# blachlylab/fade

Hardware: AMD Instinct MI355X
Metric: annotate reads/sec at 1/2/4/8 MI355X; rs/am tag bit-exact vs ref (higher is better)
Workload: dtype int16; 1 GPU; C2: 10000000 x 150 bp PE reads per GPU per step in 10 distinct batches, -w 100, --min-length 5, p_softclip 0.10; slots_in_flight=2, records_left_out=none

## Files before the change

### fade_amd/csrc/fadehip.hip

```cpp
#include "fadehip_host.hpp"
#include "fadehip_kernels.hpp"
#include "sw_stats.hpp"
#include <fcntl.h>
#include <sys/stat.h>
#include <unistd.h>
#include <algorithm>
#include <cerrno>
#include <climits>
#include <cstdio>
#include <cstdlib>
#include <cstring>
#include <string>
#include <thread>
#include <vector>

using namespace fadehip;
using namespace fadehip::host;

namespace {

int reserve_run(fadehip_ctx *ctx, std::vector<void *> &trash, DevBuf &b, size_t bytes) {
    if (bytes <= b.cap && b.p) return 0;
    if (b.p) trash.push_back(b.p);
    b.p = nullptr;
// ... 83 lines not shown
    return 0;
}

constexpr int SW_INT32 = -1;
template <int C = 0>
const void *sw_kernel(int cls, int mode, bool longw) {
    if constexpr (C >= NUM_CLASSES) {
        return nullptr;
    } else {
        if (cls != C) return sw_kernel<C + 1>(cls, mode, longw);
        constexpr int R = class_rows(C);
        switch (mode) {
        case SW_INT32: return (const void *)sw_forward_kernel<R>;
        case 0: return longw ? (const void *)sw_pk_kernel<R, 0, true> : (const void *)sw_pk_kernel<R, 0>;
        case 1: return longw ? (const void *)sw_pk_kernel<R, 1, true> : (const void *)sw_pk_kernel<R, 1>;
        case 2: return longw ? (const void *)sw_pk_kernel<R, 2, true> : (const void *)sw_pk_kernel<R, 2>;
        default: return longw ? (const void *)sw_pk_kernel<R, 3, true> : (const void *)sw_pk_kernel<R, 3>;
        }
    }
}

const void *sw64_kernel(int R) {
    switch (R) {
    case 12: return (const void *)sw_forward64_kernel<12>;
    case 16: return (const void *)sw_forward64_kernel<16>;
    case 24: return (const void *)sw_forward64_kernel<24>;
    case 32: return (const void *)sw_forward64_kernel<32>;
    case 48: return (const void *)sw_forward64_kernel<48>;
    default: return (const void *)sw_forward64_kernel<64>;
    }
}

template <int R8>
const void *g8_pick(const fadehip_ctx *ctx, int steps, bool *framed) {
    const ScoreTab &sc = ctx->sc;
    *framed = ctx->score_frame && frame_fits(std::max(std::max(sc.match, sc.mismatch), 0), sc.open, sc.ext, 8 * R8, steps);
    return *framed ? (const void *)sw_pk_kernel<R8, 1, false, 8, false, 0, true> : (const void *)sw_pk_kernel<R8, 1, false, 8>;
}
const void *g8_kernel(const fadehip_ctx *ctx, int cls, int max_lq, int steps, bool *framed) {
    const int score_g8 = ctx->score_g8, rows16 = 16 * class_rows(cls);
    *framed = false;
    if (!score_g8 || max_lq > rows16) return nullptr;
    if (max_lq <= 40 && rows16 > 40) return g8_pick<5>(ctx, steps, framed);
    if (max_lq <= 56 && rows16 > 56) return g8_pick<7>(ctx, steps, framed);
    if (max_lq <= 80 && rows16 > 80) return g8_pick<10>(ctx, steps, framed);
    if (max_lq <= 104 && rows16 > 104) return g8_pick<13>(ctx, steps, framed);
    if (max_lq <= 152 && rows16 > 152 && rows16 <= 160)
        return score_g8 == 2 ? (const void *)sw_pk_kernel<19, 1, false, 8, false, 2> : g8_pick<19>(ctx, steps, framed);
    return nullptr;
}

int launch_sw(fadehip_ctx *ctx, const void *fn, int grid, size_t lds, hipStream_t st, SwArgs a) {
    void *args[] = {&a};
    HIPCHK(ctx, hipLaunchKernel(fn, dim3((unsigned)grid), dim3(64), args, lds, st));
    return 0;
}

int resident_waves(fadehip_ctx *ctx, int cls, int mode, size_t lds, bool longw) {
    const uint64_t key = ((uint64_t)cls << 40) | ((uint64_t)mode << 32) | ((uint64_t)longw << 36) | (uint64_t)lds;
    std::lock_guard<std::mutex> l(ctx->resident_mu);
    auto it = ctx->resident.find(key);
    if (it != ctx->resident.end()) return it->second;
    int per_cu = 0;
    const void *fn = sw_kernel(cls, mode, longw);
    if (!fn || hipOccupancyMaxActiveBlocksPerMultiprocessor(&per_cu, fn, 64, lds) != hipSuccess || per_cu <= 0) per_cu = 4;
    const int w = per_cu * std::max(ctx->cu_count, 1);
    ctx->resident[key] = w;
    return w;
}

struct ClassRun {
    int cls = 0;
    const Work *work = nullptr;
    const Meta *meta = nullptr;
// ... 78 lines not shown
    p.mode2 = alt_rules ? 3 : 2;
    const int64_t ck_bytes = (int64_t)p.ck_stride * 4;
    p.total_oct = (n_items + 7) / 8;
    p.chunk_oct = std::max<int64_t>(1, std::min<int64_t>(p.total_oct, (c.budget / 2) / std::max<int64_t>(ck_bytes, 1)));
    p.wave_stride = (uint64_t)p.n_blocks1 * R * 64;
    p.longw = p.n_blocks1 > CH_BLOCKS;
    const int resident = resident_waves(ctx, cls, p.mode2, p.lds1, p.longw);
    const int bound_waves = (int)std::min<int64_t>(p.chunk_oct + NUM_BUCKETS, resident);
    int p2_waves = s.p2_last_octs[cls] >= 0 ? std::min(2 * s.p2_last_octs[cls] + 64, bound_waves) : std::min(1024, bound_waves);
    if (ctx->p2_waves_fixed > 0) p2_waves = std::min(ctx->p2_waves_fixed, bound_waves);
    p.p2_waves = (int)std::max<int64_t>(1, std::min<int64_t>(p2_waves, (c.budget / 2) / std::max<int64_t>((int64_t)p.wave_stride * 4, 1)));
    p.ckpt_bytes = (size_t)(p.chunk_oct * ck_bytes);
    p.fwd_bytes = (size_t)n_items * sizeof(Fwd);
    p.trace_bytes = (size_t)p.p2_waves * (size_t)p.wave_stride * 4;
    p.cand_bytes = sizeof(Cand) * (size_t)NUM_BUCKETS * (size_t)std::min<int64_t>(n_items, p.chunk_oct * 8);
    return 0;
}

constexpr size_t PATCH_ZB_OFF = sizeof(PatchHead), PATCH_LIST_OFF = PATCH_ZB_OFF + Slot::ZB_STRIDE;
static_assert(PATCH_LIST_OFF % 16 == 0 && Slot::ZB_BYTES % 4 == 0, "the gather copies dwords; entries stay 16-byte aligned");

int run_class_two_pass(fadehip_ctx *ctx, Slot &s, hipStream_t st, const ClassRun &c) {
    const int cls = c.cls, n_items = c.n_bound;
    TwoPassPlan p;
    int rc;
    if ((rc = plan_two_pass(ctx, s, c, p))) return rc;
    if ((rc = reserve_run(ctx, s.trash, s.ckpt, p.ckpt_bytes)) || (rc = reserve_run(ctx, s.trash, s.fwd, p.fwd_bytes)) ||
        (rc = reserve_run(ctx, s.trash, s.trace, p.trace_bytes)) || (rc = reserve_run(ctx, s.trash, s.cand, p.cand_bytes)))
        return rc;
    s.prof_counts[2] = std::max<int64_t>(s.prof_counts[2], (int64_t)p.trace_bytes);
    uint32_t *const sel_counters = s.d_sel(cls);
    const void *const score_fn = sw_kernel(cls, 1, p.longw), *const trace_fn = sw_kernel(cls, p.mode2, p.longw);
    if (!score_fn || !trace_fn) return set_err(ctx, FADEHIP_E_INVALID, "bad class %d", cls);
    bool framed = false;
    const void *const g8_fn = !p.longw && p.n_ck == 0 ? g8_kernel(ctx, cls, s.max_lq, 4 * p.n_blocks1, &framed) : nullptr;
    if (p.total_oct > p.chunk_oct) s.early = false;
    const bool early = s.early;
    for (int64_t o0 = 0; o0 < p.total_oct; o0 += p.chunk_oct) {
        const int octs = (int)std::min<int64_t>(p.chunk_oct, p.total_oct - o0);
        const int i0 = (int)(o0 * 8);
        const int n = std::min(n_items - i0, octs * 8);
        if (!s.sel_fresh[cls]) HIPCHK(ctx, hipMemsetAsync(sel_counters, 0, sizeof(uint32_t) * NUM_BUCKETS, st));
        s.sel_fresh[cls] = false;
        SwArgs a = sw_args(ctx, s, c, i0, n);
        a.ref_stride = p.ref_stride1;
        a.ckpt = (uint32_t *)s.ckpt.p;
        a.ck_stride = p.ck_stride;
        a.n_ck = p.n_ck;
        a.count_dev = c.count_dev;
        a.item_base = (uint32_t)i0;
        a.sel.enabled = 1;
        a.sel.no_ckpt = p.n_ck == 0 ? 1 : 0;
        a.sel.meta = c.meta ? c.meta + i0 : nullptr;
        a.sel.floor_len = c.floor_len;
        a.sel.trace_all = ctx->prm.trace_all;
        a.sel.span_slack = ctx->span_slack;
        a.sel.cand = (Cand *)s.cand.p;
        a.sel.cap = (uint32_t)n;
        a.sel.bucket_n = sel_counters;
        a.sel.out = c.out;
        a.sel.rs = c.rs;
        a.sel.stats = (c.rs && c.gate) ? s.d_stats() : nullptr;
        a.sel.gate = c.gate;
        a.sel.match = getenv("FADEHIP_NO_SHORTCUT") ? 0 : ctx->sc.match;
        a.sel.mismatch = ctx->sc.mismatch;
        hipStream_t sst = s.score_stream ? s.score_stream : st;
        if (sst != st) {
            int ef = -1;
            if ((rc = record(ctx, s, &ef, st))) return rc;
            HIPCHK(ctx, hipStreamWaitEvent(sst, s.ev[ef], 0));
        }
        ChunkSpans sp{c.timed};
        if ((rc = sp.mark(ctx, s, 0, sst))) return rc;
        const void *fn1 = score_fn;
        int waves1 = octs;
        size_t lds = p.lds1;
        if (ctx->score_persist && class_rows(cls) == 10 && !p.longw && s.tickets_used < (int)Slot::N_TICKETS) {
            const int res = resident_waves(ctx, cls, 1, p.lds1, p.longw);
            const int cus = std::max(ctx->cu_count, 1), mine = s.score_stream ? std::max(cus - 8 * ctx->tail_cus_per_xcd, 1) : cus;
            fn1 = (const void *)sw_pk_kernel<10, 1, false, 16, true>;
            waves1 = std::max(1, std::min(octs, (int)((int64_t)res * mine / cus)));
            a.ticket = s.d_ticket(s.tickets_used++);
        } else if (g8_fn) {
            if (ctx->debug && o0 == 0) fprintf(stderr, "[fadehip] class of %d rows: score pass on eight-lane groups (longest read of the batch: %d), column-drift frame %s\n", 16 * class_rows(cls), s.max_lq, framed ? "on" : "off");
            fn1 = g8_fn;
            waves1 = (n + 15) / 16;
            lds = 2 * p.lds1;
        }
        if ((rc = launch_sw(ctx, fn1, waves1, lds, sst, a))) return rc;
        if ((rc = sp.mark(ctx, s, 1, sst))) return rc;
        hipStream_t p2st = st;
        if (sst != st || early) {
            int ej = sp.e[1];
            if (ej < 0 && (rc = record(ctx, s, &ej, sst))) return rc;
            if (sst != st) HIPCHK(ctx, hipStreamWaitEvent(st, s.ev[ej], 0));
            if (early) {
                if (s.tail_stream) {
                    p2st = s.tail_stream;
                    HIPCHK(ctx, hipStreamWaitEvent(p2st, s.ev[ej], 0));
                }
                HIPCHK(ctx, hipMemcpyAsync(s.res.p + s.res_aln_off, s.aln.p, sizeof(fadehip_aln) * (size_t)s.out_cap, hipMemcpyDeviceToHost,
                                           s.tail_stream ? st : sst));
                HIPCHK(ctx, hipMemcpyAsync(s.res.p, c.rs, (size_t)s.n_reads, hipMemcpyDeviceToHost, s.tail_stream ? st : sst));
            }
        }
        if (s.tickets_used >= (int)Slot::N_TICKETS)
            return set_err(ctx, FADEHIP_E_UNSUPPORTED, "more than %d pass-2 launches in one run (raise trace_bytes)", (int)Slot::N_TICKETS);
        SwArgs b2 = a;
        b2.sel.enabled = 0;
        b2.n_items = 0;
        b2.cand = (const Cand *)s.cand.p;
        b2.cand_cap = (uint32_t)n;
        b2.bucket_n = sel_counters;
        b2.cand_total = &s.d_plan()->cand_total;
        b2.trace = (uint32_t *)s.trace.p;
        b2.quad_stride = p.wave_stride;
        b2.count_dev = nullptr;
// ... 1406 lines not shown
```

### fade_amd/csrc/fadehip_ctx.hip

```cpp
#include "fadehip_host.hpp"
#include <rccl/rccl.h>
#include <algorithm>
#include <cstdarg>
#include <cstdio>
#include <cstdlib>
#include <cstring>
#include <ctime>
#include <new>
#include <unordered_map>

using namespace fadehip;
using namespace fadehip::host;

namespace {

thread_local std::string g_err = "";
thread_local const fadehip_ctx *g_err_ctx = nullptr;

constexpr size_t PIN_REGISTER_MIN = (size_t)1 << 20;
std::mutex g_pin_mu;
std::unordered_map<void *, bool> g_pin_registered;

int pin_alloc(fadehip_ctx *ctx, size_t bytes, void **out) {
    *out = nullptr;
// ... 189 lines not shown
        if (atoi(kv)) {
            ctx->blocking_sync = true;
            (void)hipSetDevice(device);
            if (hipSetDeviceFlags(hipDeviceScheduleBlockingSync) != hipSuccess) (void)hipGetLastError();
        }
    }
    hipDeviceProp_t prop;
    if (hipSetDevice(device) != hipSuccess || hipGetDeviceProperties(&prop, device) != hipSuccess) {
        set_err(ctx, FADEHIP_E_NODEVICE, "cannot open HIP device %d", device);
        return fail(FADEHIP_E_NODEVICE);
    }
    if (strncmp(prop.gcnArchName, "gfx950", 6) != 0) {
        set_err(ctx, FADEHIP_E_NODEVICE, "device %d is %s; this library carries gfx950 code only", device, prop.gcnArchName);
        return fail(FADEHIP_E_NODEVICE);
    }
    ctx->cu_count = prop.multiProcessorCount;
    if (const char *kv = getenv("FADEHIP_KERNEL")) {
        ctx->use_packed = strcmp(kv, "int32") != 0;
        ctx->two_pass = strcmp(kv, "twopass") == 0;
    }
    if (ctx->prm.match > 2) ctx->two_pass = false;
    if (8 * (ctx->prm.match * FADEHIP_MAX_QUERY + ctx->prm.open + std::max(ctx->prm.match, 0)) >= 0x7c00) ctx->use_packed = false;
    if (!ctx->two_pass && ctx->prm.rules != FADEHIP_RULES_DEFAULT) {
        set_err(ctx, FADEHIP_E_UNSUPPORTED, "the rule switches exist on the two-pass path only (match <= 2, FADEHIP_KERNEL unset)");
        return fail(FADEHIP_E_UNSUPPORTED);
    }
    if (const char *kv = getenv("FADEHIP_SPAN_SLACK")) ctx->span_slack = atoi(kv);
    if (const char *kv = getenv("FADEHIP_TAIL_CUS")) ctx->tail_cus_per_xcd = std::max(0, std::min(atoi(kv), 8));
    if (const char *kv = getenv("FADEHIP_BAM_SPLIT")) ctx->split_cus = std::max(0, std::min(atoi(kv), 31));
    if (const char *kv = getenv("FADEHIP_P2_WAVES")) ctx->p2_waves_fixed = std::max(0, atoi(kv));
    if (const char *kv = getenv("FADEHIP_SCORE_PERSIST")) ctx->score_persist = atoi(kv) != 0;
    if (const char *kv = getenv("FADEHIP_SCORE_G8")) ctx->score_g8 = atoi(kv);
    if (const char *kv = getenv("FADEHIP_SCORE_FRAME")) ctx->score_frame = atoi(kv) != 0;
    if (const char *kv = getenv("FADEHIP_EARLY_COPY")) ctx->early_copy = atoi(kv) != 0;
    if (const char *kv = getenv("FADEHIP_EARLY_TAIL")) ctx->early_tail = strcmp(kv, "masked") == 0 ? 1 : strcmp(kv, "plain") == 0 ? 2 : 0;
    if (const char *kv = getenv("FADEHIP_PATCH_CAP")) ctx->patch_cap = std::max(0, std::min(atoi(kv), 1 << 20));
    ctx->debug = getenv("FADEHIP_DEBUG") != nullptr;
    if (hipStreamCreateWithFlags(&ctx->copy_stream, hipStreamNonBlocking) != hipSuccess ||
        upload_ascii_code(ctx->copy_stream) != hipSuccess) {
        set_err(ctx, FADEHIP_E_HIP, "hipMemcpyToSymbol failed: %s", hipGetErrorString(hipGetLastError()));
        return fail(FADEHIP_E_HIP);
    }
    for (int k = 0; k < FADEHIP_NUM_SLOTS; k++)
        for (int c = 0; c < NUM_CLASSES; c++) ctx->slots[k].p2_last_octs[c] = -1;
    *out = ctx;
    return 0;
}

void fadehip_destroy(fadehip_ctx *ctx) {
    if (!ctx) return;
    (void)hipSetDevice(ctx->device);
    (void)hipDeviceSynchronize();
    for (int k = 0; k < FADEHIP_NUM_SLOTS; k++) {
        Slot &s = ctx->slots[k];
        for (DevBuf *b : {&s.in[0], &s.in[1], &s.rs, &s.fwd, &s.aln, &s.zblock, &s.trace, &s.ckpt, &s.cand, &s.lrows}) release(*b);
        for (void *q : s.trash) (void)hipFree(q);
        s.trash.clear();
        for (int c = 0; c < NUM_LISTS; c++) {
            release(s.work[c]);
            release(s.meta[c]);
        }
        release(s.stage[0]);
        release(s.stage[1]);
        release(s.res);
        release(s.patch);
        release(s.h_patch);
// ... 179 lines not shown
```

### fade_amd/csrc/fadehip_host.hpp

```cpp
#pragma once
#include <hip/hip_runtime.h>
#include <climits>
#include <cstdint>
#include <map>
#include <mutex>
#include <string>
#include <vector>
#include "../../include/fadehip.h"
#include "fadehip_types.hpp"

namespace fadehip {
namespace host __attribute__((visibility("hidden"))) {

struct DevBuf {
    void *p = nullptr;
    size_t cap = 0;
};
struct PinBuf {
    uint8_t *p = nullptr;
    size_t cap = 0;
};

enum { A_TID, A_POS, A_LSEQ, A_CIGOFF, A_SEQOFF, A_FLAG, A_SA, A_CIG, A_SEQ, N_ARR };
struct Layout {
// ... 108 lines not shown
    std::mutex mu;
    hipStream_t stream = nullptr;
    DevBuf in, meta, work, out;
};

}
}

struct fadehip_ctx {
    int device = 0;
    fadehip_params prm;
    fadehip::ScoreTab sc;
    std::string err;
    std::mutex err_mu;
    fadehip::host::Slot slots[FADEHIP_NUM_SLOTS];
    fadehip::host::DevBuf genome, contig_len, contig_base;
    fadehip::host::DevBuf l1_q, l1_r, l1_qn, l1_rn, l1_bad, l1_work, l1_aln;
    hipStream_t stats_stream = nullptr;
    fadehip::host::DevBuf st_q, st_r, st_work, st_out, st_scratch;
    std::mutex stats_mu;
    fadehip::host::BatchLane batch;
    int n_contigs = 0;
    std::vector<int64_t> h_contig_len;
    std::vector<uint64_t> h_contig_base;
    int cu_count = 0;
    hipStream_t copy_stream = nullptr;
    bool use_packed = true;
    bool two_pass = true;
    int tail_cus_per_xcd = 1;
    int score_g8 = 1;
    bool blocking_sync = false;
    int split_cus = 0;
    bool score_frame = true;
    bool score_persist = false;
    int p2_waves_fixed = 0;
    bool early_copy = true;
    int early_tail = 0;
    int patch_cap = 4096;
    int span_slack = 24;
    bool debug = false;
    fadehip::host::BgzfLane bgzf[FADEHIP_BGZF_LANES];
    fadehip::host::InflateLane inf;
    bool bgzf_ready = false;
    int bgzf_geom_fixed = 0;
    double bgzf_last_ratio = 0;
    std::map<uint64_t, int> resident;
    std::mutex resident_mu;
};

#define HIPCHK(ctx, call)                                                                         \
    do {                                                                                          \
        hipError_t e_ = (call);                                                                   \
        if (e_ != hipSuccess)                                                                     \
            return fadehip::host::set_err(ctx, e_ == hipErrorOutOfMemory ? FADEHIP_E_NOMEM : FADEHIP_E_HIP,      \
                           "%s failed: %s (%s:%d)", #call, hipGetErrorString(e_), __FILE__, __LINE__); \
    } while (0)

namespace fadehip {
namespace host __attribute__((visibility("hidden"))) {

int set_err(fadehip_ctx *ctx, int code, const char *fmt, ...);
Layout batch_layout(int64_t n, int64_t n_cig, int64_t n_seq);
int reserve(fadehip_ctx *ctx, DevBuf &b, size_t bytes);
int reserve_pinned(fadehip_ctx *ctx, PinBuf &b, size_t bytes);
int reserve_roomy(fadehip_ctx *ctx, DevBuf &b, size_t bytes);
void release(DevBuf &b);
// ... 24 lines not shown
```

### fade_amd/csrc/fadehip_kernels.hpp

```cpp
#pragma once
#include <type_traits>
#include <hip/hip_runtime.h>
#include <stdint.h>
#include "../../include/fadehip.h"
#include "fadehip_types.hpp"

namespace fadehip {

__host__ __device__ constexpr uint64_t make_class_lut() {
    uint64_t v = 0;
    for (int k = 0; k < 16; k++) {
        uint64_t c = 5;
        if (k == 1) c = 0;
        if (k == 2) c = 1;
        if (k == 4) c = 2;
        if (k == 8) c = 3;
        if (k == 15) c = 4;
        v |= c << (4 * k);
    }
    return v;
}
__host__ __device__ constexpr uint64_t make_comp_lut() {
    const int t[16] = {0, 8, 4, 12, 2, 10, 6, 14, 1, 9, 5, 13, 3, 11, 7, 15};
    uint64_t v = 0;
// ... 1240 lines not shown
    return d;
}
typedef _Float16 h2v __attribute__((ext_vector_type(2)));
__device__ __forceinline__ uint32_t pk_max3_nonneg_c(uint32_t a, uint32_t b, uint32_t c) {
    const h2v m = __builtin_elementwise_maximum(__builtin_elementwise_maximum(__builtin_bit_cast(h2v, a), __builtin_bit_cast(h2v, b)), __builtin_bit_cast(h2v, c));
    return __builtin_bit_cast(uint32_t, m);
}
__device__ __forceinline__ uint32_t pk_mad4(uint32_t h, uint32_t c) {
    uint32_t d;
    asm("v_pk_mad_u16 %0, %1, 4, %2 op_sel_hi:[1,0,1]" : "=v"(d) : "v"(h), "v"(c));
    return d;
}
__device__ __forceinline__ uint32_t pk_mad8(uint32_t h, uint32_t c) {
    uint32_t d;
    asm("v_pk_mad_u16 %0, %1, 8, %2 op_sel_hi:[1,0,1]" : "=v"(d) : "v"(h), "s"(c));
    return d;
}
template <bool C>
__device__ __forceinline__ uint32_t pk_max3_sel(uint32_t a, uint32_t b, uint32_t c) {
    if constexpr (C) return pk_max3_nonneg_c(a, b, c);
    else return pk_max3_nonneg(a, b, c);
}
__device__ __forceinline__ uint32_t pk_mad_c(uint32_t h, uint32_t m, uint32_t c) { return as_u32(as_u2(h) * as_u2(m) + as_u2(c)); }
__device__ __forceinline__ uint32_t pk_mul_ffff(uint32_t a) {
    uint32_t d;
    asm("v_pk_mul_lo_u16 %0, %1, %2 op_sel_hi:[1,0]" : "=v"(d) : "v"(a), "s"(0xffffu));
    return d;
}
__device__ __forceinline__ uint32_t bfi(uint32_t mask, uint32_t a, uint32_t b) {
    uint32_t d;
    asm("v_bfi_b32 %0, %1, %2, %3" : "=v"(d) : "v"(mask), "v"(a), "v"(b));
    return d;
}

__host__ __device__ constexpr uint64_t make_cls_rc(uint32_t scale, int half) {
    uint64_t v = 0;
    for (int x = 0; x < 8; x++) {
        const uint32_t code = (uint32_t)((COMP_LUT >> (4 * (x + 8 * half))) & 15u);
        v |= (uint64_t)(scale * ((CLASS_LUT >> (4 * code)) & 15u)) << (8 * x);
    }
    return v;
}
struct ClsTab { uint64_t lo, hi; };
constexpr ClsTab CLS7_RC = {make_cls_rc(7, 0), make_cls_rc(7, 1)}, CLS16_RC = {make_cls_rc(16, 0), make_cls_rc(16, 1)};
__device__ __forceinline__ uint32_t cls4(uint32_t x, const ClsTab t) {
    const uint32_t sel = x & 0x07070707u;
    const uint32_t lo = __builtin_amdgcn_perm((uint32_t)(t.lo >> 32), (uint32_t)t.lo, sel);
    const uint32_t hi = __builtin_amdgcn_perm((uint32_t)(t.hi >> 32), (uint32_t)t.hi, sel);
    return bfi(((x >> 3) & 0x01010101u) * 0xffu, hi, lo);
}
__device__ __forceinline__ uint32_t bytes_below(int c) { return c >= 4 ? 0xffffffffu : (1u << (8 * c)) - 1u; }

constexpr int PK_SCALE = 8;

__host__ __device__ constexpr bool frame_fits(int match, int open, int ext, int rows, int steps, int lg = 8) {
    return match >= 0 && ext >= 0 && open >= ext && steps >= 0 &&
           8ll * match * rows + 8ll * ext * ((long long)steps + lg + 1) + 8ll * open + 8 * 15 < 0x7c00;
}
__host__ __device__ constexpr int pk_min_waves(int R, int MODE, int LG = 16, int WV = 0) { return WV ? WV : MODE != 1 ? 1 : (LG == 8 ? (R <= 13 ? 4 : 3) : (R <= 10 ? 4 : (R <= 16 ? 3 : 2))); }

template <int R, int MODE, bool LONGW = false, int LG = 16, bool PERSIST = false, int WV = 0, bool FRAME = false>
__global__ __launch_bounds__(64, pk_min_waves(R, MODE, LG, WV)) void sw_pk_kernel(SwArgs a) {
    static_assert(LG == 16 || (LG == 8 && MODE == 1 && !LONGW), "eight-lane groups exist for the score pass only");
    static_assert(!FRAME || (LG == 8 && MODE == 1 && !LONGW && !PERSIST), "the column-drift frame exists for the eight-lane score pass only");
    static_assert(!PERSIST || MODE == 1, "the persistent variant is a score pass");
    extern __shared__ __align__(16) uint8_t lds[];
    const int lane = threadIdx.x;
    constexpr int NG = 64 / LG, NPW = 2 * NG;
    const int g = lane / LG, lig = lane & (LG - 1);
    const uint32_t lig0m = (LG == 8 && lig == 0) ? 0xffffffffu : 0u;
    (void)lig0m;
    __shared__ uint4 wtab[49];
    if (lane < 49) {
        const int cA = lane / 7, cB = lane - 7 * cA;
        uint32_t alo = 0, ahi = 0, blo = 0, bhi = 0;
#pragma unroll
        for (int q = 0; q < 4; q++) {
            alo |= (((a.sc.prof[q] >> (4 * cA)) & 15u) * PK_SCALE) << (8 * q);
            blo |= (((a.sc.prof[q] >> (4 * cB)) & 15u) * PK_SCALE) << (8 * q);
        }
#pragma unroll
        for (int q = 4; q < 7; q++) {
            ahi |= (((a.sc.prof[q] >> (4 * cA)) & 15u) * PK_SCALE) << (8 * (q - 4));
            bhi |= (((a.sc.prof[q] >> (4 * cB)) & 15u) * PK_SCALE) << (8 * (q - 4));
        }
        wtab[lane] = make_uint4(alo, blo, ahi, bhi);
    }
    int n_items = a.n_items;
    constexpr bool P2 = (MODE >= 2);
    if constexpr (!P2) {
        if (a.count_dev) n_items = min(n_items, max(0, (int)*a.count_dev - (int)a.item_base));
    }
    for (bool first_round = true;; first_round = false) {
    int oct = blockIdx.x;
    uint32_t srcA = 0, srcB = 0, c0A = 0, c0B = 0;
    bool haveA = false, haveB = false;
    if constexpr (P2) {
        uint32_t tk = 0;
        if (lane == 0) tk = atomicAdd(a.ticket, 1u);
        oct = (int)__builtin_amdgcn_readfirstlane(tk);
        int first = 0, b = -1, local = 0, n_b = 0;
        uint32_t total = 0;
#pragma unroll
        for (int k = 0; k < NUM_BUCKETS; k++) {
            const uint32_t cnt = min(a.bucket_n[NUM_BUCKETS - 1 - k], a.cand_cap);
            const int octs_k = (int)((cnt + 7) / 8);
            if (b < 0 && oct < first + octs_k) { b = NUM_BUCKETS - 1 - k; local = oct - first; n_b = (int)cnt; }
            first += octs_k;
            total += cnt;
        }
        if (oct == 0 && lane == 0 && total && a.cand_total) atomicAdd(a.cand_total, (unsigned long long)total);
        if (b < 0) break;
        if (!first_round) __syncthreads();
        const Cand *cl = a.cand + (uint64_t)b * a.cand_cap;
        const int kA = local * 8 + g * 2, kB = kA + 1;
        if (kA < n_b) { const Cand c = cl[kA]; srcA = c.src; c0A = c.c0; haveA = true; }
        if (kB < n_b) { const Cand c = cl[kB]; srcB = c.src; c0B = c.c0; haveB = true; }
// ... 124 lines not shown
        const int shA = (srcA & 1u) ? 16 : 0, shB = (srcB & 1u) ? 16 : 0;
        auto pick = [&](int k) -> uint32_t {
            uint32_t va = 0, vb = 0;
            if (haveA && c0A) va = (ckA[k * 64] >> shA) & 0xffffu;
            if (haveB && c0B) vb = (ckB[k * 64] >> shB) & 0xffffu;
            return va | (vb << 16);
        };
#pragma unroll
        for (int r = 0; r < R; r++) {
            Hl[r] = pick(r);
            Eh[r] = pick(R + r);
        }
        hu_out = pick(2 * R);
        fu_out = pick(2 * R + 1);
        hu_prev = pick(2 * R + 2);
        uint32_t ra = PAD_CLASS, rb = PAD_CLASS;
        if (haveA && c0A) {
            const uint32_t pr = (ckA[(2 * R + 3) * 64] & 0xffffu) >> 4;
            ra = (srcA & 1u) ? pr % 7u : pr / 7u;
        }
        if (haveB && c0B) {
            const uint32_t pr = (ckB[(2 * R + 3) * 64] & 0xffffu) >> 4;
            rb = (srcB & 1u) ? pr % 7u : pr / 7u;
        }
        rc = (7u * ra + rb) * 16u;
    }
    __syncthreads();
    const uint32_t ext8 = (uint32_t)(a.sc.ext * PK_SCALE) * 0x10001u;
    const uint32_t open8 = (uint32_t)(a.sc.open * PK_SCALE) * 0x10001u;
    uint32_t fl_h = 0, fl_e = 0, kd8 = 0;
    const uint32_t oe8 = open8 - ext8, ext64 = ((uint32_t)(a.sc.ext * (8 * PK_SCALE)) & 0xffffu) * 0x10001u;
    (void)oe8; (void)ext64;
    uint32_t k8 = (uint32_t)PK_SCALE * 0x10001u;
    if constexpr (FRAME) {
        asm("" : "+s"(k8));
        fl_h = ext8 * (uint32_t)(LG - 1 - lig);
        fl_e = fl_h + oe8;
        kd8 = pk_mad_c(fl_h, k8, 0u);
#pragma unroll
        for (int r = 0; r < R; r++) Hl[r] = fl_h;
        hu_out = hu_prev = fl_h;
    }
    uint32_t *tq = a.trace + trace_off + lane;
    uint32_t *ckw = a.ckpt + (uint64_t)oct * a.ck_stride + lane;
    const uint32_t himask = __builtin_amdgcn_readfirstlane(0xffff0000u);
    const bool hdir_f_first = rule(a.sc.rules, FADEHIP_RULE_HDIR_DIAG_F_E), tie_extends = rule(a.sc.rules, FADEHIP_RULE_GAP_TIE_EXTENDS);
    const uint32_t tie_flip2 = tie_extends ? 0u : 0x00020002u, tie_flip1 = tie_extends ? 0u : 0x00010001u;
    const bool end_min_ref = rule(a.sc.rules, FADEHIP_RULE_END_MIN_REF_THEN_QUERY);
    (void)hdir_f_first; (void)tie_flip2; (void)tie_flip1; (void)end_min_ref;

    auto sweep = [&](auto fast_tag) __attribute__((always_inline)) {
    constexpr bool FAST = decltype(fast_tag)::value;
    uint32_t selA[R], selB[R];
#pragma unroll
    for (int r = 0; r < R; r++) {
        const uint32_t qa = qcls[r] & 0xffu, qb = qcls[r] >> 16;
        if constexpr (FAST) {
            selA[r] = 0x0c000c00u | (qa == PAD_CLASS ? 0x0cu : qa) | ((qb == PAD_CLASS ? 0x0cu : qb + 4u) << 16);
            selB[r] = 0;
        } else {
            selA[r] = 0x0c0c0c00u | qa;
            selB[r] = 0x0c000c0cu | (qb << 16);
        }
    }
    const uint8_t *wt = reinterpret_cast<const uint8_t *>(wtab);
    constexpr int GROUP = (MODE == 1) ? KW / 4 : (1 << 30);
    uint64_t rw_next = *reinterpret_cast<const uint64_t *>(lref);
    for (int cb = 0; cb < (LONGW ? n_blocks : 1); cb += CH_BLOCKS) {
    if constexpr (LONGW) {
        if (cb) {
            __syncthreads();
            stage(cb * 4);
            __syncthreads();
        }
    }
    const int cb_end = LONGW ? min(n_blocks, cb + CH_BLOCKS) : n_blocks;
    for (int blk0 = cb; blk0 < cb_end; blk0 += GROUP) {
    const int blk_end = (MODE == 1) ? min(cb_end, blk0 + GROUP) : cb_end;
    for (int blk = blk0; blk < blk_end; blk++) {
        uint64_t rw;
        if constexpr (MODE == 1) {
            rw = rw_next;
            rw_next = *reinterpret_cast<const uint64_t *>(lref + (min(blk + 1, n_blocks - 1) - cb) * 4);
        } else {
            rw = *reinterpret_cast<const uint64_t *>(lref + (blk - cb) * 4);
        }
        uint32_t acc[R];
        if constexpr (MODE != 1) {
#pragma unroll
            for (int k = 0; k < R; k++) acc[k] = 0;
        }
#pragma unroll
        for (int s = 0; s < 4; s++) {
            const int t = blk * 4 + s;
            const uint32_t fresh = (uint32_t)(rw >> (16 * s)) & 0xffffu;
            rc = (uint32_t)__builtin_amdgcn_update_dpp((int)fresh, (int)rc, DPP_ROW_SHR1, 0xf, 0xf, false);
            uint32_t hu = (uint32_t)__builtin_amdgcn_update_dpp(0, (int)hu_out, DPP_ROW_SHR1, 0xf, 0xf, true);
            uint32_t fu = (uint32_t)__builtin_amdgcn_update_dpp(0, (int)fu_out, DPP_ROW_SHR1, 0xf, 0xf, true);
            if constexpr (FRAME) {
                fl_h += ext8;
                fl_e += ext8;
                kd8 = as_u32(as_u2(kd8) + as_u2(ext64));
            }
            if constexpr (LG == 8) {
                rc = bfi(lig0m, fresh, rc);
                if constexpr (FRAME) hu = bfi(lig0m, fl_h, hu);
                else hu &= ~lig0m;
                fu &= ~lig0m;
            }
            uint2 tA, tB;
            if constexpr (FAST) {
                const uint2 e = *reinterpret_cast<const uint2 *>(wt + rc);
                tA.x = e.x;
                tB.x = e.y;
                tA.y = tB.y = 0;
            } else {
                const uint4 e = *reinterpret_cast<const uint4 *>(wt + rc);
                tA = make_uint2(e.x, e.z);
                tB = make_uint2(e.y, e.w);
            }
            const uint32_t ct = (uint32_t)(0xffff - t);
            const uint32_t tk = (uint32_t)(KW - 1 - (t & (KW - 1))) * 0x10001u;
            const uint32_t tk_even = end_min_ref ? tk * 2u + 0x10001u : tk + (uint32_t)KW * 0x10001u, tk_odd = end_min_ref ? tk * 2u : tk;
            uint32_t tkf_even = 0, tkf_odd = 0;
            if constexpr (FRAME) {
                tkf_even = as_u32(as_u2(tk_even) - as_u2(kd8));
                tkf_odd = as_u32(as_u2(tk_odd) - as_u2(kd8));
            }
            (void)tkf_even; (void)tkf_odd;
            uint32_t kprev = 0;
            uint32_t hd = hu_prev;
            hu_prev = hu;
#pragma unroll
            for (int r = 0; r < R; r++) {
                uint32_t Dp;
                if constexpr (FAST) {
                    Dp = hd + __builtin_amdgcn_perm(tB.x, tA.x, selA[r]);
                } else {
                    const uint32_t wA = __builtin_amdgcn_perm(tA.y, tA.x, selA[r]);
                    const uint32_t wB = __builtin_amdgcn_perm(tB.y, tB.x, selB[r]);
                    Dp = hd + wA + wB;
                }
                const uint32_t hl = Hl[r];
                uint32_t Ee = 0, Fe = 0, En, Fn, T, H;
                if constexpr (FRAME) {
                    En = pk_max3_nonneg_c(hl, Eh[r], fl_e);
                    Fn = as_u32(__builtin_elementwise_max(as_s2(hu), as_s2(fu)) - as_s2(ext8));
                    T = pk_max3_nonneg_c(Dp, En, Fn);
                    H = as_u32(as_s2(T) - as_s2(oe8));
                } else {
                    Ee = as_u32(as_s2(Eh[r]) - as_s2(ext8));
                    En = as_u32(__builtin_elementwise_max(as_s2(hl), as_s2(Ee)));
                    Fe = as_u32(as_s2(fu) - as_s2(ext8));
                    Fn = as_u32(__builtin_elementwise_max(as_s2(hu), as_s2(Fe)));
                    T = pk_max3_nonneg(Dp, En, Fn);
                    H = as_u32(__builtin_elementwise_sub_sat(as_u2(T), as_u2(open8)));
                }
                (void)Ee; (void)Fe;
                if constexpr (MODE != 1) {
                    const uint32_t m1 = pk_min_k<8>(pk_sub(T, Dp));
                    uint32_t m2, m3, m4;
                    if constexpr (MODE == 3) {
                        m2 = pk_min_k<4>(pk_sub(T, hdir_f_first ? Fn : En));
                        m3 = pk_min_k<2>(pk_sub(En, tie_extends ? Ee : hl)) ^ tie_flip2;
                        m4 = pk_min_k<1>(pk_sub(Fn, tie_extends ? Fe : hu)) ^ tie_flip1;
                    } else {
                        m2 = pk_min_k<4>(pk_sub(T, Fn));
                        m3 = pk_min_k<2>(pk_sub(En, Ee));
                        m4 = pk_min_k<1>(pk_sub(Fn, Fe));
                    }
                    uint32_t &ac = acc[(r - s + R) % R];
                    ac = pk_shl4_add(ac, m1) + m2 + m3 + m4;
                }
                if constexpr (MODE == 0) {
                    bestA[r] = max(bestA[r], (H << 16) | ct);
                    bestB[r] = max(bestB[r], and_or(H, himask, ct));
                }
                if constexpr (MODE == 1 && !PAIRKEY) {
// ... 49 lines not shown
#pragma unroll
            for (int r = 0; r < R; r++) {
                cp[r * 64] = Hl[r];
                cp[(R + r) * 64] = Eh[r];
            }
            cp[(2 * R) * 64] = hu_out;
            cp[(2 * R + 1) * 64] = fu_out;
            cp[(2 * R + 2) * 64] = hu_prev;
            cp[(2 * R + 3) * 64] = rc;
        }
    }
    }
    }
    };
    if (__any(special)) sweep(std::false_type{});
    else sweep(std::true_type{});

    constexpr int NK = PAIRKEY ? (R + 1) / 2 : R;
    uint32_t rowA[R], rowB[R];
#pragma unroll
    for (int r = 0; r < R; r++) { rowA[r] = (uint32_t)r; rowB[r] = (uint32_t)r; }
    if constexpr (MODE == 1 && !PAIRKEY) {
#pragma unroll
        for (int r = 0; r < R; r++) {
            const uint32_t gh = bestB[r], gt = GT[r];
            const uint32_t ha = (gh & 0xffffu) >> 2, hb = gh >> 18;
            bestA[r] = ha ? ((ha << 16) | (0xffffu - (gt & 0xffffu))) : 0u;
            bestB[r] = hb ? ((hb << 16) | (0xffffu - (gt >> 16))) : 0u;
        }
    }
    if constexpr (PAIRKEY) {
#pragma unroll
        for (int p2 = 0; p2 < NK; p2++) {
            const uint32_t gh = bestB[p2], gt = GT[p2];
            constexpr int KS = KLOW - 3, KB = KLOW - 1;
            const uint32_t ha = ((gh & 0xffffu) >> KLOW) << 3, hb = (gh >> (16 + KLOW)) << 3;
            static_assert(KS == 2 || KS == 3, "key scale");
            const uint32_t gta = gt & 0xffffu, gtb = gt >> 16;
            const uint32_t ta = end_min_ref ? gta >> 1 : ((gta >> KLOW) << KB) | (gta & (uint32_t)(KW - 1));
            const uint32_t tb = end_min_ref ? gtb >> 1 : ((gtb >> KLOW) << KB) | (gtb & (uint32_t)(KW - 1));
            rowA[p2] = 2u * (uint32_t)p2 + (end_min_ref ? (gta & 1u) : ((gta >> KB) & 1u));
            rowB[p2] = 2u * (uint32_t)p2 + (end_min_ref ? (gtb & 1u) : ((gtb >> KB) & 1u));
            bestA[p2] = ha ? ((ha << 16) | (0xffffu - ta)) : 0u;
            bestB[p2] = hb ? ((hb << 16) | (0xffffu - tb)) : 0u;
        }
    }
    if constexpr (!P2) {
        uint32_t bka = 0, bkb = 0;
        int browa = 0, browb = 0;
#pragma unroll
        for (int r = 0; r < NK; r++) {
            const int ra = lig * R + (int)rowA[r], rb = lig * R + (int)rowB[r];
            const uint32_t ka = end_min_ref ? bestA[r] : (bestA[r] & 0xffff0000u), kb = end_min_ref ? bestB[r] : (bestB[r] & 0xffff0000u);
            if (ra < lqA && ka > (end_min_ref ? bka : (bka & 0xffff0000u))) { bka = bestA[r]; browa = ra; }
            if (rb < lqB && kb > (end_min_ref ? bkb : (bkb & 0xffff0000u))) { bkb = bestB[r]; browb = rb; }
        }
        uint64_t ca = 0, cb = 0;
        if (bka >> 16) {
            const uint64_t h = bka >> 16, nj = (bka + (uint32_t)lig) & 0xffffu, ni = (uint64_t)(0xffff - browa);
            ca = end_min_ref ? (h << 32) | (nj << 16) | ni : (h << 32) | (ni << 16) | nj;
        }
        if (bkb >> 16) {
            const uint64_t h = bkb >> 16, nj = (bkb + (uint32_t)lig) & 0xffffu, ni = (uint64_t)(0xffff - browb);
            cb = end_min_ref ? (h << 32) | (nj << 16) | ni : (h << 32) | (ni << 16) | nj;
        }
#pragma unroll
        for (int m = 1; m < LG; m <<= 1) {
// ... 269 lines not shown
```

Baseline: 1.310 billion reads/s.

## Add row-and-step drift frame variant to eight-lane score pass

Adds a DIAG variant of the framed g8 score kernel. It folds the gap-extension penalty into the substitution profile and into a per-row, per-step offset, so the inner loop drops the per-cell F extension subtraction and the per-step frame increments. The key and tie values are corrected at the end by subtracting the accumulated per-row drift. The host picks this variant by default whenever the new diag_fits bound holds. It adds range constraints on the int16 packed scores and more complex key reconstruction, which risks breaking bit-exactness.

```diff
diff --git a/fade_amd/csrc/fadehip.hip b/fade_amd/csrc/fadehip.hip
--- a/fade_amd/csrc/fadehip.hip
+++ b/fade_amd/csrc/fadehip.hip
@@ -139,14 +139,16 @@
 }
 
 template <int R8>
-const void *g8_pick(const fadehip_ctx *ctx, int steps, bool *framed) {
+const void *g8_pick(const fadehip_ctx *ctx, int steps, int *framed) {
     const ScoreTab &sc = ctx->sc;
-    *framed = ctx->score_frame && frame_fits(std::max(std::max(sc.match, sc.mismatch), 0), sc.open, sc.ext, 8 * R8, steps);
-    return *framed ? (const void *)sw_pk_kernel<R8, 1, false, 8, false, 0, true> : (const void *)sw_pk_kernel<R8, 1, false, 8>;
-}
-const void *g8_kernel(const fadehip_ctx *ctx, int cls, int max_lq, int steps, bool *framed) {
+    const int match = std::max(std::max(sc.match, sc.mismatch), 0);
+    *framed = !ctx->score_frame ? 0 : ctx->score_diag && diag_fits(match, sc.open, sc.ext, 8 * R8, steps) ? 2 : frame_fits(match, sc.open, sc.ext, 8 * R8, steps) ? 1 : 0;
+    return *framed == 2 ? (const void *)sw_pk_kernel<R8, 1, false, 8, false, 0, true, true>
+           : *framed ? (const void *)sw_pk_kernel<R8, 1, false, 8, false, 0, true> : (const void *)sw_pk_kernel<R8, 1, false, 8>;
+}
+const void *g8_kernel(const fadehip_ctx *ctx, int cls, int max_lq, int steps, int *framed) {
     const int score_g8 = ctx->score_g8, rows16 = 16 * class_rows(cls);
-    *framed = false;
+    *framed = 0;
     if (!score_g8 || max_lq > rows16) return nullptr;
     if (max_lq <= 40 && rows16 > 40) return g8_pick<5>(ctx, steps, framed);
     if (max_lq <= 56 && rows16 > 56) return g8_pick<7>(ctx, steps, framed);
@@ -291,7 +293,7 @@
     uint32_t *const sel_counters = s.d_sel(cls);
     const void *const score_fn = sw_kernel(cls, 1, p.longw), *const trace_fn = sw_kernel(cls, p.mode2, p.longw);
     if (!score_fn || !trace_fn) return set_err(ctx, FADEHIP_E_INVALID, "bad class %d", cls);
-    bool framed = false;
+    int framed = 0;
     const void *const g8_fn = !p.longw && p.n_ck == 0 ? g8_kernel(ctx, cls, s.max_lq, 4 * p.n_blocks1, &framed) : nullptr;
     if (p.total_oct > p.chunk_oct) s.early = false;
     const bool early = s.early;
@@ -341,7 +343,7 @@
             waves1 = std::max(1, std::min(octs, (int)((int64_t)res * mine / cus)));
             a.ticket = s.d_ticket(s.tickets_used++);
         } else if (g8_fn) {
-            if (ctx->debug && o0 == 0) fprintf(stderr, "[fadehip] class of %d rows: score pass on eight-lane groups (longest read of the batch: %d), column-drift frame %s\n", 16 * class_rows(cls), s.max_lq, framed ? "on" : "off");
+            if (ctx->debug && o0 == 0) fprintf(stderr, "[fadehip] class of %d rows: score pass on eight-lane groups (longest read of the batch: %d), column-drift frame %s, row drift %s\n", 16 * class_rows(cls), s.max_lq, framed ? "on" : "off", framed == 2 ? "on" : "off");
             fn1 = g8_fn;
             waves1 = (n + 15) / 16;
             lds = 2 * p.lds1;
diff --git a/fade_amd/csrc/fadehip_ctx.hip b/fade_amd/csrc/fadehip_ctx.hip
--- a/fade_amd/csrc/fadehip_ctx.hip
+++ b/fade_amd/csrc/fadehip_ctx.hip
@@ -245,6 +245,7 @@
     if (const char *kv = getenv("FADEHIP_SCORE_PERSIST")) ctx->score_persist = atoi(kv) != 0;
     if (const char *kv = getenv("FADEHIP_SCORE_G8")) ctx->score_g8 = atoi(kv);
     if (const char *kv = getenv("FADEHIP_SCORE_FRAME")) ctx->score_frame = atoi(kv) != 0;
+    if (const char *kv = getenv("FADEHIP_SCORE_DIAG")) ctx->score_diag = atoi(kv) != 0;
     if (const char *kv = getenv("FADEHIP_EARLY_COPY")) ctx->early_copy = atoi(kv) != 0;
     if (const char *kv = getenv("FADEHIP_EARLY_TAIL")) ctx->early_tail = strcmp(kv, "masked") == 0 ? 1 : strcmp(kv, "plain") == 0 ? 2 : 0;
     if (const char *kv = getenv("FADEHIP_PATCH_CAP")) ctx->patch_cap = std::max(0, std::min(atoi(kv), 1 << 20));
diff --git a/fade_amd/csrc/fadehip_host.hpp b/fade_amd/csrc/fadehip_host.hpp
--- a/fade_amd/csrc/fadehip_host.hpp
+++ b/fade_amd/csrc/fadehip_host.hpp
@@ -164,6 +164,7 @@
     bool blocking_sync = false;
     int split_cus = 0;
     bool score_frame = true;
+    bool score_diag = true;
     bool score_persist = false;
     int p2_waves_fixed = 0;
     bool early_copy = true;
diff --git a/fade_amd/csrc/fadehip_kernels.hpp b/fade_amd/csrc/fadehip_kernels.hpp
--- a/fade_amd/csrc/fadehip_kernels.hpp
+++ b/fade_amd/csrc/fadehip_kernels.hpp
@@ -1296,6 +1296,11 @@
     asm("v_bfi_b32 %0, %1, %2, %3" : "=v"(d) : "v"(mask), "v"(a), "v"(b));
     return d;
 }
+__device__ __forceinline__ uint32_t bfi_s(uint32_t mask, uint32_t a, uint32_t b) {
+    uint32_t d;
+    asm("v_bfi_b32 %0, %1, %2, %3" : "=v"(d) : "v"(mask), "s"(a), "v"(b));
+    return d;
+}
 
 __host__ __device__ constexpr uint64_t make_cls_rc(uint32_t scale, int half) {
     uint64_t v = 0;
@@ -1321,10 +1326,19 @@
     return match >= 0 && ext >= 0 && open >= ext && steps >= 0 &&
            8ll * match * rows + 8ll * ext * ((long long)steps + lg + 1) + 8ll * open + 8 * 15 < 0x7c00;
 }
+constexpr int DIAG_C0 = 2;
+__host__ __device__ constexpr bool diag_fits(int match, int open, int ext, int rows, int steps, int lg = 8) {
+    const int R = rows / lg;
+    return match >= 0 && ext >= 0 && open >= ext && steps >= 0 &&
+           8ll * match * rows + 8ll * ext * ((long long)steps + R - 1 + DIAG_C0) + 8ll * open + 8 * (15 + ext) < 0x7c00 &&
+           64ll * match * rows + 63 + 128ll * ext * (R - 1) / 2 < 0x7c00 &&
+           8 * (15 + ext) <= 255;
+}
 __host__ __device__ constexpr int pk_min_waves(int R, int MODE, int LG = 16, int WV = 0) { return WV ? WV : MODE != 1 ? 1 : (LG == 8 ? (R <= 13 ? 4 : 3) : (R <= 10 ? 4 : (R <= 16 ? 3 : 2))); }
 
-template <int R, int MODE, bool LONGW = false, int LG = 16, bool PERSIST = false, int WV = 0, bool FRAME = false>
+template <int R, int MODE, bool LONGW = false, int LG = 16, bool PERSIST = false, int WV = 0, bool FRAME = false, bool DIAG = false>
 __global__ __launch_bounds__(64, pk_min_waves(R, MODE, LG, WV)) void sw_pk_kernel(SwArgs a) {
+    static_assert(!DIAG || FRAME, "the row-and-step drift is a variant of the framed sweep");
     static_assert(LG == 16 || (LG == 8 && MODE == 1 && !LONGW), "eight-lane groups exist for the score pass only");
     static_assert(!FRAME || (LG == 8 && MODE == 1 && !LONGW && !PERSIST), "the column-drift frame exists for the eight-lane score pass only");
     static_assert(!PERSIST || MODE == 1, "the persistent variant is a score pass");
@@ -1347,6 +1361,12 @@
         for (int q = 4; q < 7; q++) {
             ahi |= (((a.sc.prof[q] >> (4 * cA)) & 15u) * PK_SCALE) << (8 * (q - 4));
             bhi |= (((a.sc.prof[q] >> (4 * cB)) & 15u) * PK_SCALE) << (8 * (q - 4));
+        }
+        if constexpr (DIAG) {
+            const uint32_t e8 = (uint32_t)(a.sc.ext * PK_SCALE);
+            constexpr uint32_t HI_REAL = (1u << (8 * (PAD_CLASS - 4))) - 1u;
+            if (cA != PAD_CLASS) { alo += e8 * 0x01010101u; ahi += e8 * (0x01010101u & HI_REAL); }
+            if (cB != PAD_CLASS) { blo += e8 * 0x01010101u; bhi += e8 * (0x01010101u & HI_REAL); }
         }
         wtab[lane] = make_uint4(alo, blo, ahi, bhi);
     }
@@ -1537,7 +1557,17 @@
     const uint32_t oe8 = open8 - ext8, ext64 = ((uint32_t)(a.sc.ext * (8 * PK_SCALE)) & 0xffffu) * 0x10001u;
     (void)oe8; (void)ext64;
     uint32_t k8 = (uint32_t)PK_SCALE * 0x10001u;
-    if constexpr (FRAME) {
+    uint32_t hand8 = ext8 * (uint32_t)(R - 1);
+    (void)hand8;
+    if constexpr (DIAG) {
+        asm("" : "+v"(k8));
+        asm("" : "+v"(hand8));
+#pragma unroll
+        for (int r = 0; r < R; r++) Hl[r] = ext8 * (uint32_t)(r + DIAG_C0 - 1);
+        hu_out = ext8 * (uint32_t)(R - 1 + DIAG_C0 - 1);
+        hu_prev = ext8 * (uint32_t)(DIAG_C0 - 2);
+        fu_out = hand8;
+    } else if constexpr (FRAME) {
         asm("" : "+s"(k8));
         fl_h = ext8 * (uint32_t)(LG - 1 - lig);
         fl_e = fl_h + oe8;
@@ -1553,6 +1583,8 @@
     const uint32_t tie_flip2 = tie_extends ? 0u : 0x00020002u, tie_flip1 = tie_extends ? 0u : 0x00010001u;
     const bool end_min_ref = rule(a.sc.rules, FADEHIP_RULE_END_MIN_REF_THEN_QUERY);
     (void)hdir_f_first; (void)tie_flip2; (void)tie_flip1; (void)end_min_ref;
+    const uint32_t dk_mul = end_min_ref ? 2u : 1u, dk_even = end_min_ref ? 1u : (uint32_t)KW, e64 = (uint32_t)(a.sc.ext * (8 * PK_SCALE));
+    (void)dk_mul; (void)dk_even; (void)e64;
 
     auto sweep = [&](auto fast_tag) __attribute__((always_inline)) {
     constexpr bool FAST = decltype(fast_tag)::value;
@@ -1602,14 +1634,18 @@
             rc = (uint32_t)__builtin_amdgcn_update_dpp((int)fresh, (int)rc, DPP_ROW_SHR1, 0xf, 0xf, false);
             uint32_t hu = (uint32_t)__builtin_amdgcn_update_dpp(0, (int)hu_out, DPP_ROW_SHR1, 0xf, 0xf, true);
             uint32_t fu = (uint32_t)__builtin_amdgcn_update_dpp(0, (int)fu_out, DPP_ROW_SHR1, 0xf, 0xf, true);
-            if constexpr (FRAME) {
+            if constexpr (DIAG) {
+                hu -= hand8;
+                fu -= hand8;
+            } else if constexpr (FRAME) {
                 fl_h += ext8;
                 fl_e += ext8;
                 kd8 = as_u32(as_u2(kd8) + as_u2(ext64));
             }
             if constexpr (LG == 8) {
                 rc = bfi(lig0m, fresh, rc);
-                if constexpr (FRAME) hu = bfi(lig0m, fl_h, hu);
+                if constexpr (DIAG) hu = bfi_s(lig0m, ext8 * (uint32_t)(t + DIAG_C0 - 1), hu);
+                else if constexpr (FRAME) hu = bfi(lig0m, fl_h, hu);
                 else hu &= ~lig0m;
                 fu &= ~lig0m;
             }
@@ -1628,7 +1664,11 @@
             const uint32_t tk = (uint32_t)(KW - 1 - (t & (KW - 1))) * 0x10001u;
             const uint32_t tk_even = end_min_ref ? tk * 2u + 0x10001u : tk + (uint32_t)KW * 0x10001u, tk_odd = end_min_ref ? tk * 2u : tk;
             uint32_t tkf_even = 0, tkf_odd = 0;
-            if constexpr (FRAME) {
+            if constexpr (DIAG) {
+                const uint32_t pos = (uint32_t)(KW - 1 - (t & (KW - 1))) * dk_mul;
+                tkf_even = ((pos + dk_even - e64 * (uint32_t)(t + DIAG_C0)) & 0xffffu) * 0x10001u;
+                tkf_odd = ((pos - e64 * (uint32_t)(t + DIAG_C0 + 1)) & 0xffffu) * 0x10001u;
+            } else if constexpr (FRAME) {
                 tkf_even = as_u32(as_u2(tk_even) - as_u2(kd8));
                 tkf_odd = as_u32(as_u2(tk_odd) - as_u2(kd8));
             }
@@ -1648,7 +1688,13 @@
                 }
                 const uint32_t hl = Hl[r];
                 uint32_t Ee = 0, Fe = 0, En, Fn, T, H;
-                if constexpr (FRAME) {
+                if constexpr (DIAG) {
+                    const uint32_t fl = oe8 + ext8 * (uint32_t)(t + r + DIAG_C0);
+                    En = pk_max3_nonneg_c(hl, Eh[r], fl);
+                    Fn = as_u32(__builtin_elementwise_max(as_s2(hu), as_s2(fu)));
+                    T = pk_max3_nonneg_c(Dp, En, Fn);
+                    H = as_u32(as_s2(T) - as_s2(oe8));
+                } else if constexpr (FRAME) {
                     En = pk_max3_nonneg_c(hl, Eh[r], fl_e);
                     Fn = as_u32(__builtin_elementwise_max(as_s2(hu), as_s2(fu)) - as_s2(ext8));
                     T = pk_max3_nonneg_c(Dp, En, Fn);
@@ -1764,7 +1810,9 @@
     if constexpr (PAIRKEY) {
 #pragma unroll
         for (int p2 = 0; p2 < NK; p2++) {
-            const uint32_t gh = bestB[p2], gt = GT[p2];
+            uint32_t gh = bestB[p2];
+            const uint32_t gt = GT[p2];
+            if constexpr (DIAG) gh = pk_sub(gh, (((uint32_t)(a.sc.ext * 128 * p2)) & 0xffffu) * 0x10001u);
             constexpr int KS = KLOW - 3, KB = KLOW - 1;
             const uint32_t ha = ((gh & 0xffffu) >> KLOW) << 3, hb = (gh >> (16 + KLOW)) << 3;
             static_assert(KS == 2 || KS == 3, "key scale");
```

New measurement: 1.463 billion reads/s, median of 6. +11.7%, better.
